# TheDisorderedOrganization/MonteCarlo

Hardware: AMD Instinct MI355X
Metric: chain-updates/sec (MC sweeps x M) at M=10^7 per MI355X (higher is better)
Workload: dtype f64

## Files before the change

montecarlo_amd/csrc/amc_api.hip:

```cpp
#include "amc_internal.h"

static thread_local std::string g_last_error;

int fail(int code, const char* fmt, ...)
{
    char buf[2048];
    va_list ap;
    va_start(ap, fmt);
    vsnprintf(buf, sizeof(buf), fmt, ap);
    va_end(ap);
    g_last_error = buf;
    return code;
}

int grid_for(const amc_handle* h, int64_t n_items, int blocks_per_cu)
{
    int64_t blocks = (n_items + AMC_BLOCK - 1) / AMC_BLOCK;
    const int64_t cap = (int64_t)h->n_cu * (blocks_per_cu > 0 ? blocks_per_cu : h->blocks_per_cu);
    if (blocks > cap) blocks = cap;
    if (blocks < 1) blocks = 1;
    return (int)blocks;
}

static int push_params(amc_handle* h, const double* sigma, const double* weight)
// ... 231 lines not shown
        if (e != hipErrorNotReady) return e;
        if ((spins & 63) == 63) {
            timespec t1;
            clock_gettime(CLOCK_MONOTONIC, &t1);
            if ((t1.tv_sec - t0.tv_sec) * 1000000000ll + (t1.tv_nsec - t0.tv_nsec) > 5000000ll) break;
        }
    }
    return hipStreamSynchronize(stream);
}

static hipError_t wait_event(hipEvent_t ev)
{
    timespec t0;
    clock_gettime(CLOCK_MONOTONIC, &t0);
    for (int spins = 0;; ++spins) {
        const hipError_t e = hipEventQuery(ev);
        if (e != hipErrorNotReady) return e;
        if ((spins & 63) == 63) {
            timespec t1;
            clock_gettime(CLOCK_MONOTONIC, &t1);
            if ((t1.tv_sec - t0.tv_sec) * 1000000000ll + (t1.tv_nsec - t0.tv_nsec) > 5000000ll) break;
        }
    }
    return hipEventSynchronize(ev);
}


extern "C" {

const char* amc_last_error(void) { return g_last_error.c_str(); }

int amc_version(void) { return AMC_VERSION_MAJOR * 1000 + AMC_VERSION_MINOR; }

int amc_device_count(int* count)
{
    if (!count) return fail(AMC_ERR_BAD_ARG, "amc_device_count: count is NULL");
    int n = 0;
    hipError_t e = hipGetDeviceCount(&n);
    if (e != hipSuccess) { *count = 0; return fail(AMC_ERR_NO_DEVICE, "hipGetDeviceCount: %s", hipGetErrorString(e)); }
    *count = n;
    return AMC_OK;
}

struct ClassExprs { const char *sample, *logq, *dlogq, *perform, *invert; };
struct ProposalExprs { const char *sample, *logq, *dlogq, *perform, *invert; int n_params; const char* const* dlogq_more;
                       int n_classes; const ClassExprs* more_classes; const int* class_of_move; };

static int validate_proposal_exprs(const ProposalExprs* proposal)
{
    int rc_p = validate_potential_expr(proposal->sample, "sample_action expression", "z");
    if (rc_p == AMC_OK) rc_p = validate_potential_expr(proposal->logq, "log_proposal_density expression", "delta");
    if (rc_p == AMC_OK && proposal->dlogq) {
        rc_p = validate_potential_expr(proposal->dlogq, "d log_proposal_density / d sigma expression", proposal->n_params > 1 ? "" : "sigma");
        if (rc_p != AMC_OK && proposal->n_params == 1 &&
            validate_potential_expr(proposal->dlogq, "d log_proposal_density / d sigma expression", "theta0") == AMC_OK)
            rc_p = AMC_OK;
    }
    for (int pidx = 1; rc_p == AMC_OK && proposal->dlogq && pidx < proposal->n_params; ++pidx)
        rc_p = validate_potential_expr(proposal->dlogq_more[pidx - 1], "d log_proposal_density / d theta expression", "");
    if (rc_p == AMC_OK && (proposal->perform != nullptr) != (proposal->invert != nullptr))
        rc_p = fail(AMC_ERR_BAD_ARG, "amc_create_action_model: perform_expr and invert_expr come together (No invert_action! is defined)");
    if (rc_p == AMC_OK && proposal->perform) rc_p = validate_potential_expr(proposal->perform, "perform_action expression", "delta");
    if (rc_p == AMC_OK && proposal->invert) rc_p = validate_potential_expr(proposal->invert, "invert_action expression", "delta");
    for (int c = 1; rc_p == AMC_OK && c < proposal->n_classes; ++c) {
        const ClassExprs& ce = proposal->more_classes[c - 1];
        rc_p = validate_potential_expr(ce.sample, "sample_action expression", "z");
// ... 85 lines not shown
    }
    if (std::fabs(wsum - 1.0) > 1.4901161193847656e-08)
        return fail(AMC_ERR_BAD_ARG, "amc_create: weights must sum to 1 (got %.17g)", wsum);
    if (cfg->n_moves > 1 && !cfg->per_chain_counters) {
    }

    int n_dev = 0;
    hipError_t e = hipGetDeviceCount(&n_dev);
    if (e != hipSuccess || n_dev < 1)
        return fail(AMC_ERR_NO_DEVICE, "amc_create: no HIP device (%s); this engine has no CPU path",
                    e != hipSuccess ? hipGetErrorString(e) : "count = 0");
    if (cfg->device < 0 || cfg->device >= n_dev)
        return fail(AMC_ERR_BAD_ARG, "amc_create: device %d out of range [0, %d)", cfg->device, n_dev);
    AMC_HIP(hipSetDevice(cfg->device));
    hipDeviceProp_t prop;
    AMC_HIP(hipGetDeviceProperties(&prop, cfg->device));

    amc_handle* h = new (std::nothrow) amc_handle();
    if (!h) return fail(AMC_ERR_OOM, "amc_create: host allocation failed");
    h->device = cfg->device;
    h->n_cu = prop.multiProcessorCount > 0 ? prop.multiProcessorCount : 256;
    {
        std::string arch(prop.gcnArchName);
        const size_t colon = arch.find(':');
        if (colon != std::string::npos) arch.erase(colon);
        if (!arch.empty()) h->arch = arch;
        if (h->arch != AMC_BUILD_ARCH) {
            delete h;
            return fail(AMC_ERR_NO_DEVICE, "amc_create: device %d is %s, this libamc.so was built for %s (make ARCH=%s)", cfg->device,
                        arch.c_str(), AMC_BUILD_ARCH, arch.c_str());
        }
    }
    h->blocks_per_cu = 8;
    h->blocks_per_cu_single = (cfg->n_moves == 1 && !cfg->per_chain_counters) ? 6 : (cfg->n_moves > 1 ? 7 : 8);
    if (const char* env = std::getenv("AMC_BLOCKS_PER_CU")) {
        const int v = std::atoi(env);
        if (v >= 1 && v <= 64) h->blocks_per_cu = h->blocks_per_cu_single = h->blocks_per_cu_pg = v;
    }
    if (const char* env = std::getenv("AMC_BLOCKS_PER_CU_SINGLE")) {
        const int v = std::atoi(env);
        if (v >= 1 && v <= 64) h->blocks_per_cu_single = v;
    }
    if (const char* env = std::getenv("AMC_BLOCKS_PER_CU_REDUCE")) {
        const int v = std::atoi(env);
        if (v >= 1 && v <= 64) h->blocks_per_cu_red = v;
    }
    if (const char* env = std::getenv("AMC_EXACT_ACCEPT")) h->exact_accept = std::atoi(env) != 0;
    if (const char* env = std::getenv("AMC_WIDE_RED_ROWS")) h->wide_red_rows = std::atoi(env) != 0;
    if (const char* env = std::getenv("AMC_SHARD_ROUTE_ON_ONE_RANK")) h->shard_route_one_rank = std::atoi(env) != 0;
    if (const char* env = std::getenv("AMC_NO_DEFERRED_UPDATE")) h->no_deferred_update = std::atoi(env) != 0;
    if (const char* env = std::getenv("AMC_CLASS_PER_MOVE")) h->class_per_move_forced = std::atoi(env) != 0;
    if (const char* env = std::getenv("AMC_NO_COLUMN_SKIP")) h->no_column_skip = std::atoi(env) != 0;
    if (const char* env = std::getenv("AMC_NP_SMALL_LAUNCHES")) h->np_small_launches = std::atoi(env) != 0;
    h->M = cfg->n_chains;
    h->M_pad = ((cfg->n_chains + AMC_PAD_DOUBLES + 255) / 256) * 256;
    h->offset = cfg->chain_offset;
    h->M_global = cfg->n_chains_global;
    h->potential = cfg->potential;
    h->f32 = state_dtype == AMC_DTYPE_F32;
    h->use_rtc = h->f32 || cfg->potential == AMC_POTENTIAL_CUSTOM;
    h->pot_expr = encode_model_expr(h->f32, potential_expr, reward_expr, scale_expr, proposal);
    if (potential_expr && scale_expr) h->scaled_policy = true;
    if (potential_expr && proposal) {
        if (proposal->n_classes > 1) {
            h->n_classes = proposal->n_classes;
            for (int k = 0; k < cfg->n_moves; ++k) h->class_of_move[k] = proposal->class_of_move[k];
        }
        h->script_policy = true;
        h->script_dlogq = proposal->dlogq != nullptr;
        h->n_params = proposal->n_params;
    }
    h->K = cfg->n_moves;
    h->sweepstep = cfg->sweepstep;
    h->counters = cfg->per_chain_counters != 0 || cfg->n_moves > 1;
    h->beta = cfg->beta;
    h->seed = cfg->seed;

    int rc = AMC_OK;
    auto bail = [&](int code) { amc_destroy(h); return code; };
#define AMC_TRY(call)                                                                   \
    do {                                                                                \
        hipError_t e2_ = (call);                                                        \
        if (e2_ != hipSuccess) {                                                        \
            rc = fail(e2_ == hipErrorOutOfMemory ? AMC_ERR_OOM : AMC_ERR_HIP,           \
                      "%s failed: %s", #call, hipGetErrorString(e2_));                  \
            return bail(rc);                                                            \
        }                                                                               \
    } while (0)

    if (cfg->stream) {
        h->stream = (hipStream_t)cfg->stream;
    } else {
        AMC_TRY(hipStreamCreateWithFlags(&h->stream, hipStreamNonBlocking));
// ... 1218 lines not shown
```

montecarlo_amd/csrc/amc_math.h:

```cpp
#pragma once

#ifndef __HIPCC_RTC__
#include <hip/hip_runtime.h>
#include <stdint.h>
#else
typedef unsigned char uint8_t;
typedef unsigned short uint16_t;
typedef int int32_t;
typedef unsigned int uint32_t;
typedef long int64_t;
typedef unsigned long uint64_t;
#endif

#include "amc_tables.h"

namespace amc {

enum : uint32_t { STREAM_INIT = 0, STREAM_METROPOLIS = 1, STREAM_ESTIMATOR = 2 };
enum : uint32_t { DRAW_NORMAL = 0, DRAW_ACCEPT = 1 };

struct u32x4 { uint32_t x, y, z, w; };

__device__ __forceinline__ void stage_math_tables(double* lds, int tid, int nthreads)
{
    for (int i = tid; i < TAB_DOUBLES; i += nthreads) {
        const double v = AMC_MATH_TABLES[i];
        lds[i] = (i >= TAB_LOG_LOGC && i < TAB_SINPI) ? -2.0 * v : v;
    }
    __syncthreads();
}

__device__ __forceinline__ u32x4 philox4x32_10(u32x4 c, uint32_t k0, uint32_t k1)
{
#pragma unroll
    for (int r = 0; r < 10; ++r) {
        const uint64_t m0 = (uint64_t)0xD2511F53u * c.x;
        const uint64_t m1 = (uint64_t)0xCD9E8D57u * c.z;
        u32x4 n;
        n.x = __builtin_amdgcn_bitop3_b32((uint32_t)(m1 >> 32), c.y, k0, 0x96);
        n.y = (uint32_t)m1;
        n.z = __builtin_amdgcn_bitop3_b32((uint32_t)(m0 >> 32), c.w, k1, 0x96);
        n.w = (uint32_t)m0;
        c = n;
        k0 += 0x9E3779B9u;
        k1 += 0xBB67AE85u;
#ifndef AMC_PHILOX_HOISTED_KEYS
        asm volatile("" : "+s"(k0), "+s"(k1));
#endif
    }
    return c;
}

__device__ __forceinline__ u32x4 draw_counter(uint64_t pair, uint64_t t, uint32_t draw, uint32_t stream)
{
    u32x4 c;
    c.x = (uint32_t)t;
    c.y = ((uint32_t)(t >> 32) & 0xFFFFu) | ((draw & 0xFFFu) << 16) | ((stream & 0xFu) << 28);
    c.z = (uint32_t)pair;
    c.w = (uint32_t)(pair >> 32);
    return c;
}

__device__ __forceinline__ double bits_to_binade(uint32_t lo, uint32_t hi, uint32_t expo_hi)
{
    const uint32_t w_hi = __builtin_amdgcn_alignbit(expo_hi, hi, 12);
    const uint32_t w_lo = __builtin_amdgcn_alignbit(hi, lo, 12);
    return __longlong_as_double((long long)(((uint64_t)w_hi << 32) | w_lo));
}

__device__ __forceinline__ double uniform_co(uint32_t lo, uint32_t hi) { return bits_to_binade(lo, hi, 0x3FFu) - 1.0; }
__device__ __forceinline__ double uniform_oc(uint32_t lo, uint32_t hi) { return 2.0 - bits_to_binade(lo, hi, 0x3FFu); }
__device__ __forceinline__ double angle28(uint32_t w)
{
    const uint32_t w_hi = __builtin_amdgcn_alignbit(0x400u, w, 12);
    const uint32_t w_lo = (w << 20) & 0xFF000000u;
    return 4.0 - __longlong_as_double((long long)(((uint64_t)w_hi << 32) | w_lo));
}

__device__ __forceinline__ uint32_t spare_accept12(const u32x4& n, int half) { return half ? ((n.z >> 12) & 0xFFFu) : (n.x & 0xFFFu); }
__device__ __forceinline__ uint32_t spare_pick12(const u32x4& n, int half) { return half ? ((n.z >> 24) | ((n.w & 0xFu) << 8)) : (n.z & 0xFFFu); }
__device__ __forceinline__ double uniform_accept(uint32_t accept12, uint32_t lo, uint32_t hi)
{
    const uint32_t w_hi = 0x3FF00000u | (accept12 << 8) | (hi >> 24);
    const uint32_t w_lo = __builtin_amdgcn_alignbit(hi, lo, 24);
    return __longlong_as_double((long long)(((uint64_t)w_hi << 32) | w_lo)) - 1.0;
}
__device__ __forceinline__ double uniform_pick(uint32_t pick12, uint32_t lo)
{
    return (double)(((uint64_t)pick12 << 24) | (uint64_t)(lo & 0xFFFFFFu)) * 0x1.0p-36;
}

__device__ __forceinline__ double exp_core_f64(double x, const double* T)
{
    const double INV_L = 0x1.71547652b82fep+5;
    const double L_HI = 0x1.62e42fee00000p-6;
    const double L_LO = 0x1.a39ef35793c76p-38;
    const double SHIFT = 0x1.8p52;
    const double t = __builtin_fma(x, INV_L, SHIFT);
    const double kd = t - SHIFT;
    const int32_t ki = (int32_t)(uint32_t)(uint64_t)__double_as_longlong(t);
    double r = __builtin_fma(-kd, L_HI, x);
    r = __builtin_fma(-kd, L_LO, r);
    double p = 0x1.6c16c16c16c17p-10;
    p = __builtin_fma(p, r, 0x1.1111111111111p-7);
    p = __builtin_fma(p, r, 0x1.5555555555555p-5);
    p = __builtin_fma(p, r, 0x1.5555555555555p-3);
    p = __builtin_fma(p, r, 0x1.0000000000000p-1);
    p = __builtin_fma(p, r, 1.0);
    p = __builtin_fma(p, r, 1.0);
    const double y = T[TAB_EXP2 + (ki & 31)] * p;
    const int32_t m = ki >> 5;
    const uint64_t yb = (uint64_t)__double_as_longlong(y);
    const uint32_t yh = (uint32_t)(yb >> 32) + ((uint32_t)m << 20);
    return __longlong_as_double((long long)(((uint64_t)yh << 32) | (yb & 0xffffffffull)));
}

__device__ __forceinline__ double exp_f64(double x, const double* T)
{
    double y = exp_core_f64(x, T);
    y = (x < -708.0) ? 0.0 : y;
    y = (x > 709.0) ? __builtin_huge_val() : y;
    y = (x != x) ? x : y;
    return y;
}

__device__ __forceinline__ double log_f64(double x)
{
    const double LN2_HI = 0x1.62e42fee00000p-1;
    const double LN2_LO = 0x1.a39ef35793c76p-33;
    const double x0 = x;
    int64_t k = 0;
    uint64_t ux = (uint64_t)__double_as_longlong(x);
    if (ux < 0x0010000000000000ull) {
        x = x * 0x1.0p54;
        ux = (uint64_t)__double_as_longlong(x);
        k = -54;
    }
    uint32_t hx = (uint32_t)(ux >> 32);
    k += (int64_t)(hx >> 20) - 1023;
// ... 123 lines not shown
```

montecarlo_amd/csrc/amc_model.h:

```cpp
#pragma once

#include "amc_math.h"
#include "amc_xsum.h"

#define AMC_MAX_MOVES 64
#define AMC_MAX_LEARN 8
#ifndef AMC_BLOCK
#define AMC_BLOCK 256
#endif
#define AMC_PAD_DOUBLES (2 * AMC_BLOCK + 8)

namespace amc {

enum { POT_HARMONIC = 0, POT_DOUBLE_WELL = 1, POT_CUSTOM = 2 };

#ifndef AMC_PLAIN_KERNELS
#define AMC_PLAIN_KERNELS 1
#endif
#ifndef AMC_KERNEL_LINKAGE
#define AMC_KERNEL_LINKAGE
#endif

#ifdef AMC_STATE_F32
typedef float real_t;
// ... 322 lines not shown
#endif
}
#endif
#undef amc_exp
#undef amc_log

template <int POT>
__device__ __forceinline__ real_t potential(real_t x, const double* T)
{
    if (POT == POT_CUSTOM) return user_potential(x, T);
    if (POT == POT_DOUBLE_WELL) {
        const real_t q = x * x - (real_t)1.0;
        return q * q;
    }
    return x * x;
}

struct Proposal {
    real_t delta, xn, dlogp;
};

template <int POT>
__device__ __forceinline__ Proposal propose(real_t x, real_t beta, double sigma, double z, const double* T)
{
    Proposal p;
    p.delta = (real_t)__builtin_fma(sigma, z, 0.0);
    const real_t e1 = potential<POT>(x, T);
    p.xn = x + p.delta;
    const real_t e2 = potential<POT>(p.xn, T);
    p.dlogp = ((-e2) * beta) - ((-e1) * beta);
    return p;
}

__device__ __forceinline__ bool accept_exact(real_t delta, real_t dlogp, double den, double rden, double logc, double u,
                                             const double* T)
{
    const double logq = div_by_const((double)(-(delta * delta)), den, rden) - logc;
    const double arg = ((double)dlogp + logq) - logq;
    const bool c_pos = arg >= 0.0, c_rng = arg >= -708.0, c_exp = exp_core_f64(arg, T) > u;
    return c_pos | (c_rng & c_exp);
}

#define AMC_FILTER_EPS 0x1.0p-16f
struct FilterCmp {
    bool pos, lo, hi;
};

__device__ __forceinline__ FilterCmp accept_filter(real_t dlogp, uint32_t k)
{
    const float t = (float)dlogp;
    const float ex = __builtin_amdgcn_exp2f(__builtin_fmaxf(t, -17.0f) * 0x1.715476p+0f);
    const float kf = (float)k;
    constexpr float SCALE = 4096.0f;
    const float lo1 = __builtin_fmaf(ex, (1.0f - AMC_FILTER_EPS) * SCALE, -1.0f);
    const float hi = ex * ((1.0f + AMC_FILTER_EPS) * SCALE);
    FilterCmp c;
    c.pos = t > 2e-12f;
    c.lo = lo1 > kf;
    c.hi = hi < kf;
    return c;
}

__device__ __forceinline__ FilterCmp accept_filter_arg(double arg, uint32_t k)
{
    const float t = (float)arg;
    const float ex = __builtin_amdgcn_exp2f(__builtin_fmaxf(t, -17.0f) * 0x1.715476p+0f);
    const float kf = (float)k;
    constexpr float SCALE = 4096.0f;
    const float lo1 = __builtin_fmaf(ex, (1.0f - AMC_FILTER_EPS) * SCALE, -1.0f);
    const float hi = ex * ((1.0f + AMC_FILTER_EPS) * SCALE);
    FilterCmp c;
    c.pos = arg >= 0.0;
// ... 116 lines not shown
            if (!have_pu) {
                asm volatile("" : "+v"(accept_ctr.z));
                pu = philox4x32_10(accept_ctr, key0, key1);
            }
            a0 = accept_exact_arg(s0.arg, uniform_accept(a0_12, pu.x, pu.y), T);
            a1 = accept_exact_arg(s1.arg, uniform_accept(a1_12, pu.z, pu.w), T);
        }
        xv.x = a0 ? s0.xn : s0.xr;
        xv.y = a1 ? s1.xn : s1.xr;
        m0 = __builtin_amdgcn_ballot_w64(a0);
        m1_out = __builtin_amdgcn_ballot_w64(a1);
        acc_bits = (a0 ? 1u : 0u) | (a1 ? 0x100u : 0u);
        return;
    }
#endif
    const Proposal p0 = propose<POT>(xv.x, b0, sg0, z0, T), p1 = propose<POT>(xv.y, b1, sg1, z1, T);
    const real_t xr0 = p0.xn + (-p0.delta), xr1 = p1.xn + (-p1.delta);
    const FilterCmp c0 = accept_filter(p0.dlogp, a0_12), c1 = accept_filter(p1.dlogp, a1_12);
#define AMC_B(c) __builtin_amdgcn_ballot_w64(c)
    const unsigned long long acc0 = AMC_B(c0.pos) | AMC_B(c0.lo), rej0 = AMC_B(c0.hi);
    const unsigned long long acc1 = AMC_B(c1.pos) | AMC_B(c1.lo), rej1 = AMC_B(c1.hi);
    const unsigned long long undecided = AMC_B(true) & ~((acc0 | rej0) & (acc1 | rej1));
#undef AMC_B
    if ((undecided | force_mask) != 0ull) {
        if (!have_pu) {
            asm volatile("" : "+v"(accept_ctr.z));
            pu = philox4x32_10(accept_ctr, key0, key1);
        }
        MoveExact e0 = m1, e1 = m1;
        if (MULTI) {
            e0.dn = s_tab[AMC_MAX_MOVES + k0]; e0.lc = s_tab[2 * AMC_MAX_MOVES + k0]; e0.rd = s_tab[4 * AMC_MAX_MOVES + k0];
            e1.dn = s_tab[AMC_MAX_MOVES + k1]; e1.lc = s_tab[2 * AMC_MAX_MOVES + k1]; e1.rd = s_tab[4 * AMC_MAX_MOVES + k1];
        }
        const bool a0 = accept_exact(p0.delta, p0.dlogp, e0.dn, e0.rd, e0.lc, uniform_accept(a0_12, pu.x, pu.y), T);
        const bool a1 = accept_exact(p1.delta, p1.dlogp, e1.dn, e1.rd, e1.lc, uniform_accept(a1_12, pu.z, pu.w), T);
        m0 = __builtin_amdgcn_ballot_w64(a0);
        m1_out = __builtin_amdgcn_ballot_w64(a1);
        xv.x = a0 ? p0.xn : xr0;
        xv.y = a1 ? p1.xn : xr1;
        acc_bits = (a0 ? 1u : 0u) | (a1 ? 0x100u : 0u);
    } else {
        const bool a0 = c0.pos | c0.lo, a1 = c1.pos | c1.lo;
        m0 = acc0;
        m1_out = acc1;
        xv.x = a0 ? p0.xn : xr0;
        xv.y = a1 ? p1.xn : xr1;
        acc_bits = (a0 ? 1u : 0u) | (a1 ? 0x100u : 0u);
    }
}

typedef uint32_t u32v4_t __attribute__((ext_vector_type(4)));

typedef uint32_t u32v2_t __attribute__((ext_vector_type(2)));

__device__ __forceinline__ real2 load_pair_block(const real_t* block_base)
{
    const __amdgpu_buffer_rsrc_t r = __builtin_amdgcn_make_buffer_rsrc((void*)block_base, 0, 0x7fffffff, 0x00020000);
    real2 d;
#ifdef AMC_STATE_F32
    const u32v2_t v = __builtin_amdgcn_raw_buffer_load_b64(r, threadIdx.x * 8, 0, 0);
    d.x = __uint_as_float(v.x);
    d.y = __uint_as_float(v.y);
#else
    const u32v4_t v = __builtin_amdgcn_raw_buffer_load_b128(r, threadIdx.x * 16, 0, 0);
    d.x = __longlong_as_double((long long)(((uint64_t)v.y << 32) | v.x));
    d.y = __longlong_as_double((long long)(((uint64_t)v.w << 32) | v.z));
#endif
    return d;
// ... 16 lines not shown
```

montecarlo_amd/csrc/amc_sweep.h:

```cpp
#pragma once

#include "amc_wave_sums.h"

namespace amc {

struct SweepArgs {
    real_t* x;
    const real_t* beta_arr;
    uint8_t* log;
    const double* ptab;
    const uint8_t* pick_tab;
    unsigned long long* acc_total;
    int64_t n_chains;
    int64_t m_stride;
    uint64_t pair0;
    uint64_t t0;
    int32_t n_steps;
    int32_t n_moves;
    uint32_t key0, key1;
    double beta;
    xs_word* red_partials;
    int32_t red_stride;
    int32_t red_cols;
    int32_t log_pos;
    int32_t exact_accept;
    int32_t n_slots;
};

struct StepDraws {
    u32x4 normal;
};

__device__ __forceinline__ StepDraws step_draws(const SweepArgs& a, uint64_t pair, uint64_t t)
{
    StepDraws d;
    d.normal = philox4x32_10(draw_counter(pair, t, DRAW_NORMAL, STREAM_METROPOLIS), a.key0, a.key1);
    return d;
// ... 52 lines not shown
        const u32x4 accept_ctr = draw_counter(pair, t, DRAW_ACCEPT, STREAM_METROPOLIS);
        double sg0 = sigma1, sg1 = sigma1;
        int k0 = 0, k1 = 0;
        u32x4 pu = {0u, 0u, 0u, 0u};
        bool have_pu = false;
        if (MULTI) {
            const uint32_t q0 = spare_pick12(dr.normal, 0), q1 = spare_pick12(dr.normal, 1);
            k0 = s_pick[q0];
            k1 = s_pick[q1];
            const bool open = ((k0 | k1) & 0x80) != 0;
            if ((__builtin_amdgcn_ballot_w64(open) | force_mask) != 0ull) {
                pu = philox4x32_10(accept_ctr, a.key0, a.key1);
                have_pu = true;
                k0 = categorical_walk(s_tab, K, uniform_pick(q0, pu.x));
                k1 = categorical_walk(s_tab, K, uniform_pick(q1, pu.z));
            }
            sg0 = s_tab[k0];
            sg1 = s_tab[k1];
        }
        double z0, z1;
        box_muller(dr.normal, z0, z1, s_math, mk);
        unsigned long long m0, m1m;
        uint32_t acc_bits;
        mh_pair<POT, MULTI>(xv, b0, b1, sg0, sg1, k0, k1, s_tab, m1, z0, z1, dr.normal, pu, have_pu, accept_ctr, a.key0,
                            a.key1, s_math, force_mask, acc_bits, m0, m1m, th1);
        if (!MULTI) wave_acc += __popcll(m0 & __builtin_amdgcn_ballot_w64(v0)) + __popcll(m1m & __builtin_amdgcn_ballot_w64(v1));
        if (LOG) {
            log_word = acc_bits | ((uint32_t)k0 << 1) | ((uint32_t)k1 << 9);
            if (!SINGLE && v0) store_log_pair<LOG>(a, a.log_pos + s, p, log_word);
        }
    }
}

template <int POT, bool MULTI, int LOG, bool BETA, bool SINGLE, int REDUCE = RED_FORM_NONE>
__global__ __launch_bounds__(AMC_BLOCK) void sweep_kernel(const SweepArgs a)
{
    static_assert(!MULTI || LOG, "K > 1 always keeps per-chain counters");
    constexpr bool RED_E = REDUCE == RED_FORM_E;
    constexpr int RNC = RedCols<POT, RED_E>::NC;
    RLanes<RNC> red;
    __shared__ xs::PartR s_red[REDUCE ? AMC_BLOCK / 64 : 1][RNC];
    if (REDUCE) r_init(red, s_red[threadIdx.x >> 6]);
    __shared__ double s_tab[MULTI ? (5 + AMC_SIGMA_MEMO) * AMC_MAX_MOVES : 1];
    __shared__ __attribute__((aligned(16))) uint8_t s_pick[MULTI ? AMC_PICK_CELLS : 16];
    __shared__ double s_math[TAB_DOUBLES];
    const int K = a.n_moves;
    if (MULTI) {
        stage_pick_table(s_pick, a.pick_tab);
        for (int i = threadIdx.x; i < K; i += AMC_BLOCK) {
            s_tab[0 * AMC_MAX_MOVES + i] = a.ptab[PT_SIGMA * AMC_MAX_MOVES + i];
            s_tab[1 * AMC_MAX_MOVES + i] = a.ptab[PT_DEN * AMC_MAX_MOVES + i];
            s_tab[2 * AMC_MAX_MOVES + i] = a.ptab[PT_LOGC * AMC_MAX_MOVES + i];
            s_tab[3 * AMC_MAX_MOVES + i] = a.ptab[PT_CUM * AMC_MAX_MOVES + i];
            s_tab[4 * AMC_MAX_MOVES + i] = a.ptab[PT_RDEN * AMC_MAX_MOVES + i];
            if (AMC_SIGMA_MEMO) s_tab[(AMC_SIGMA_MEMO ? 5 : 0) * AMC_MAX_MOVES + i] = log_f64(a.ptab[PT_SIGMA * AMC_MAX_MOVES + i]);
        }
    }
    const double sigma1 = a.ptab[PT_SIGMA * AMC_MAX_MOVES];
    const double den1 = a.ptab[PT_DEN * AMC_MAX_MOVES];
    const double logc1 = a.ptab[PT_LOGC * AMC_MAX_MOVES];
    const double rden1 = a.ptab[PT_RDEN * AMC_MAX_MOVES];
    UserTheta th1 = {0.0, 0.0, 0.0, 0.0, 0.0, 0.0};
#ifdef AMC_USER_LOGQ
    if (!MULTI) th1 = user_theta_uniform(a.ptab, 0);
#endif

    const int64_t n_pairs = (a.n_chains + 1) >> 1;
    const int64_t stride = (int64_t)gridDim.x * AMC_BLOCK;
    const int64_t first = (int64_t)blockIdx.x * AMC_BLOCK;
    unsigned long long wave_acc = 0;
    unsigned long long slots_before = 0;
    if (REDUCE && !LOG && !MULTI && threadIdx.x == 0)
        for (int sl = (int)blockIdx.x; sl < a.n_slots; sl += (int)gridDim.x) slots_before += a.acc_total[sl];

    auto load_x = [&](int64_t b) -> real2 { return load_pair_block(a.x + 2 * b); };
    auto load_b = [&](int64_t b) -> real2 { return load_pair_block(a.beta_arr + 2 * b); };
    real2 x_nxt = {(real_t)0.0, (real_t)0.0}, b_nxt = {(real_t)a.beta, (real_t)a.beta};
    if (first < n_pairs) {
        x_nxt = load_x(first);
        if (BETA) b_nxt = load_b(first);
    }
    constexpr bool AHEAD = SINGLE;
    StepDraws dr_nxt = {};
    if (AHEAD && first < n_pairs) dr_nxt = step_draws(a, a.pair0 + (uint64_t)(first + threadIdx.x), a.t0);
#ifdef AMC_USER_LOGQ
    stage_user_theta(a.ptab, MULTI);
#endif
    stage_math_tables(s_math, threadIdx.x, AMC_BLOCK);
    __builtin_amdgcn_s_waitcnt(0x0F70);
    real2 x_done = {(real_t)0.0, (real_t)0.0};
    uint32_t lw_done = 0;
    int64_t base_done = -1;
    int64_t base = first;
    for (; base + stride < n_pairs; base += stride) {
        const int64_t p = base + threadIdx.x;
        real2 xv = x_nxt;
        const real_t b0 = b_nxt.x, b1 = b_nxt.y;
        x_nxt = load_x(base + stride);
        if (BETA) b_nxt = load_b(base + stride);
        if (base_done >= 0) {
            store_pair_block_writethrough(a.x + 2 * base_done, x_done);
            if (LOG && SINGLE) store_log_pair<LOG>(a, a.log_pos, base_done + threadIdx.x, lw_done);
        }
        const StepDraws dr = dr_nxt;
        uint32_t lw = 0;
        pair_steps<POT, MULTI, LOG, SINGLE, AHEAD>(a, xv, b0, b1, a.pair0 + (uint64_t)p, p, true, true, s_tab, s_pick, s_math,
                                                   sigma1, den1, rden1, logc1, wave_acc, lw, &dr, math_k_literal(), th1);
        if (AHEAD) dr_nxt = step_draws(a, a.pair0 + (uint64_t)(p + stride), a.t0);
        if (REDUCE) {
            red_add_pair<POT, RED_E>(red, xv, true, true, s_math, s_red[threadIdx.x >> 6], a.red_cols);
        }
        x_done = xv;
        lw_done = lw;
        base_done = base;
    }
    if (base < n_pairs) {
        const int64_t p = base + threadIdx.x;
        const bool v0 = p < n_pairs;
        const bool v1 = v0 && (2 * p + 1 < a.n_chains);
        real2 xv = x_nxt;
        if (base_done >= 0) {
            store_pair_block_writethrough(a.x + 2 * base_done, x_done);
            if (LOG && SINGLE) store_log_pair<LOG>(a, a.log_pos, base_done + threadIdx.x, lw_done);
        }
        uint32_t lw = 0;
        pair_steps<POT, MULTI, LOG, SINGLE, AHEAD>(a, xv, b_nxt.x, b_nxt.y, a.pair0 + (uint64_t)(v0 ? p : 0), p, v0, v1,
                                                   s_tab, s_pick, s_math, sigma1, den1, rden1, logc1, wave_acc, lw, &dr_nxt, math_k_literal(), th1);
        if (v0) {
            store_pair_block_writethrough(a.x + 2 * base, xv);
            if (LOG && SINGLE) store_log_pair<LOG>(a, a.log_pos, p, lw);
        }
        if (REDUCE) red_add_pair<POT, RED_E>(red, xv, v0, v1, s_math, s_red[threadIdx.x >> 6], a.red_cols);
    }
    if (REDUCE)
        red_finish<POT, RED_E>(red, s_red, a.red_partials + (int64_t)blockIdx.x * a.red_stride, a.red_stride == RED_COMPACT_WORDS, a.red_cols);
    if (!MULTI) {
        __shared__ unsigned long long s_acc[AMC_BLOCK / 64];
        if ((threadIdx.x & 63) == 0) s_acc[threadIdx.x >> 6] = wave_acc;
        __syncthreads();
        if (threadIdx.x == 0) {
            unsigned long long t = 0;
            for (int w = 0; w < AMC_BLOCK / 64; ++w) t += s_acc[w];
            if (REDUCE && !LOG) {
                if (t != 0) __hip_atomic_fetch_add(a.acc_total + blockIdx.x, t, __ATOMIC_RELAXED, __HIP_MEMORY_SCOPE_AGENT);
                a.red_partials[(int64_t)blockIdx.x * a.red_stride + (a.red_stride == RED_COMPACT_WORDS ? (int)RED_COMPACT_SLOT : (int)RED_ROW_SLOT)] =
                    (xs_word)__double_as_longlong((double)(slots_before + t));
            } else if (t != 0) {
                __hip_atomic_fetch_add(a.acc_total + blockIdx.x, t, __ATOMIC_RELAXED, __HIP_MEMORY_SCOPE_AGENT);
            }
        }
    }
}

__device__ __forceinline__ unsigned long long add_block_accepts(unsigned long long* acc_total, unsigned long long wave_acc)
{
    __shared__ unsigned long long s_acc2[AMC_BLOCK / 64];
    if ((threadIdx.x & 63) == 0) s_acc2[threadIdx.x >> 6] = wave_acc;
    __syncthreads();
    unsigned long long t = 0;
    if (threadIdx.x == 0) {
        for (int w = 0; w < AMC_BLOCK / 64; ++w) t += s_acc2[w];
        if (t != 0) __hip_atomic_fetch_add(acc_total + blockIdx.x, t, __ATOMIC_RELAXED, __HIP_MEMORY_SCOPE_AGENT);
    }
    __syncthreads();
    return t;
}

#define AMC_FOLD_TILE (16 * AMC_BLOCK)
__device__ __forceinline__ uint4 load_counter_quad(const uint32_t* p) { return *reinterpret_cast<const uint4*>(p); }
__device__ __forceinline__ uint4 load_counter_quad(const uint16_t* p)
{
    const uint2 v = *reinterpret_cast<const uint2*>(p);
    return uint4{v.x & 0xFFFFu, v.x >> 16, v.y & 0xFFFFu, v.y >> 16};
}
__device__ __forceinline__ void store_counter_quad(uint32_t* p, uint4 v) { *reinterpret_cast<uint4*>(p) = v; }
__device__ __forceinline__ void store_counter_quad(uint16_t* p, uint4 v)
{
    *reinterpret_cast<uint2*>(p) = uint2{v.x | (v.y << 16), v.z | (v.w << 16)};
}

template <bool HIGH, typename CT>
__device__ __forceinline__ uint4 bump_counter_quad(CT* lo, uint16_t* hi, uint32_t w)
{
    uint4 v = load_counter_quad(lo);
// ... 172 lines not shown
```

montecarlo_amd/csrc/amc_tables.h:

```cpp
#pragma once
#ifndef __HIPCC_RTC__
#include <hip/hip_runtime.h>
#endif
namespace amc {
enum { TAB_EXP2 = 0, TAB_LOG_INVC = 32, TAB_LOG_LOGC = 161, TAB_SINPI = 290, TAB_COSPI = 418,
       TAB_DOUBLES = 546, TAB_LOG_IDX_MIN = 53 };
__device__ const double AMC_MATH_TABLES[546] = {
    0x1.0000000000000p+0, 0x1.059b0d3158574p+0, 0x1.0b5586cf9890fp+0, 0x1.11301d0125b51p+0,
    0x1.172b83c7d517bp+0, 0x1.1d4873168b9aap+0, 0x1.2387a6e756238p+0, 0x1.29e9df51fdee1p+0,
    0x1.306fe0a31b715p+0, 0x1.371a7373aa9cbp+0, 0x1.3dea64c123422p+0, 0x1.44e086061892dp+0,
    0x1.4bfdad5362a27p+0, 0x1.5342b569d4f82p+0, 0x1.5ab07dd485429p+0, 0x1.6247eb03a5585p+0,
    0x1.6a09e667f3bcdp+0, 0x1.71f75e8ec5f74p+0, 0x1.7a11473eb0187p+0, 0x1.82589994cce13p+0,
    0x1.8ace5422aa0dbp+0, 0x1.93737b0cdc5e5p+0, 0x1.9c49182a3f090p+0, 0x1.a5503b23e255dp+0,
    0x1.ae89f995ad3adp+0, 0x1.b7f76f2fb5e47p+0, 0x1.c199bdd85529cp+0, 0x1.cb720dcef9069p+0,
    0x1.d5818dcfba487p+0, 0x1.dfc97337b9b5fp+0, 0x1.ea4afa2a490dap+0, 0x1.f50765b6e4540p+0,
    0x1.6900000000000p+0, 0x1.6700000000000p+0, 0x1.6500000000000p+0, 0x1.6300000000000p+0,
    0x1.6180000000000p+0, 0x1.5f80000000000p+0, 0x1.5d80000000000p+0, 0x1.5b80000000000p+0,
    0x1.5a00000000000p+0, 0x1.5800000000000p+0, 0x1.5600000000000p+0, 0x1.5480000000000p+0,
    0x1.5280000000000p+0, 0x1.5100000000000p+0, 0x1.4f00000000000p+0, 0x1.4d80000000000p+0,
    0x1.4c00000000000p+0, 0x1.4a00000000000p+0, 0x1.4880000000000p+0, 0x1.4700000000000p+0,
    0x1.4500000000000p+0, 0x1.4380000000000p+0, 0x1.4200000000000p+0, 0x1.4080000000000p+0,
    0x1.3f00000000000p+0, 0x1.3d80000000000p+0, 0x1.3c00000000000p+0, 0x1.3a80000000000p+0,
    0x1.3900000000000p+0, 0x1.3780000000000p+0, 0x1.3600000000000p+0, 0x1.3480000000000p+0,
    0x1.3300000000000p+0, 0x1.3180000000000p+0, 0x1.3000000000000p+0, 0x1.2e80000000000p+0,
    0x1.2d80000000000p+0, 0x1.2c00000000000p+0, 0x1.2a80000000000p+0, 0x1.2900000000000p+0,
    0x1.2800000000000p+0, 0x1.2680000000000p+0, 0x1.2500000000000p+0, 0x1.2400000000000p+0,
    0x1.2280000000000p+0, 0x1.2180000000000p+0, 0x1.2000000000000p+0, 0x1.1f00000000000p+0,
    0x1.1d80000000000p+0, 0x1.1c80000000000p+0, 0x1.1b00000000000p+0, 0x1.1a00000000000p+0,
    0x1.1880000000000p+0, 0x1.1780000000000p+0, 0x1.1680000000000p+0, 0x1.1500000000000p+0,
    0x1.1400000000000p+0, 0x1.1300000000000p+0, 0x1.1180000000000p+0, 0x1.1080000000000p+0,
    0x1.0f80000000000p+0, 0x1.0e80000000000p+0, 0x1.0d00000000000p+0, 0x1.0c00000000000p+0,
    0x1.0b00000000000p+0, 0x1.0a00000000000p+0, 0x1.0900000000000p+0, 0x1.0780000000000p+0,
    0x1.0680000000000p+0, 0x1.0580000000000p+0, 0x1.0480000000000p+0, 0x1.0380000000000p+0,
    0x1.0280000000000p+0, 0x1.0180000000000p+0, 0x1.0000000000000p+0, 0x1.0000000000000p+0,
    0x1.fa00000000000p-1, 0x1.f600000000000p-1, 0x1.f200000000000p-1, 0x1.ef00000000000p-1,
    0x1.eb00000000000p-1, 0x1.e700000000000p-1, 0x1.e400000000000p-1, 0x1.e000000000000p-1,
    0x1.dd00000000000p-1, 0x1.d900000000000p-1, 0x1.d600000000000p-1, 0x1.d200000000000p-1,
    0x1.cf00000000000p-1, 0x1.cc00000000000p-1, 0x1.c900000000000p-1, 0x1.c600000000000p-1,
    0x1.c200000000000p-1, 0x1.bf00000000000p-1, 0x1.bc00000000000p-1, 0x1.b900000000000p-1,
    0x1.b600000000000p-1, 0x1.b300000000000p-1, 0x1.b100000000000p-1, 0x1.ae00000000000p-1,
// ... 107 lines not shown
```

Baseline: 335.9 billion.

## Overlap math-table staging with chain loads, pin exp constants, raise residency

The kernel prologue now issues the math-table global loads as 16-byte pairs at kernel start and writes them into LDS only after the first chain/beta loads are in flight, so the table staging overlaps the initial memory latency. The first-step random draws move after the barrier. Exp-core constants in the exact-accept path are forced into scalar registers via an inline-asm barrier, and single-move sweep kernels get a waves-per-EU hint of 7, with the default blocks-per-CU for the non-RTC single case raised from 6 to 7. Optional timestamp diagnostics compiled out by default are added. Higher residency may increase register pressure or spills.

Measured after the change: 335.7 billion (median of 4 runs). Within noise of the previous version (-0.1%).

```diff
diff --git a/montecarlo_amd/csrc/amc_api.hip b/montecarlo_amd/csrc/amc_api.hip
--- a/montecarlo_amd/csrc/amc_api.hip
+++ b/montecarlo_amd/csrc/amc_api.hip
@@ -287,6 +287,19 @@
 
 int amc_version(void) { return AMC_VERSION_MAJOR * 1000 + AMC_VERSION_MINOR; }
 
+#ifdef AMC_DIAG_STAMPS
+extern "C" __attribute__((visibility("default"))) int amc_diag_stamps_read(unsigned long long* out, int clear)
+{
+    const size_t bytes = sizeof(unsigned long long) * AMC_DIAG_WAVES * AMC_DIAG_POINTS;
+    if (out && hipMemcpyFromSymbol(out, HIP_SYMBOL(amc::amc_diag_stamps), bytes, 0, hipMemcpyDeviceToHost) != hipSuccess) return -1;
+    if (clear) {
+        void* p = nullptr;
+        if (hipGetSymbolAddress(&p, HIP_SYMBOL(amc::amc_diag_stamps)) != hipSuccess || hipMemset(p, 0, bytes) != hipSuccess) return -1;
+    }
+    return AMC_DIAG_WAVES * AMC_DIAG_POINTS;
+}
+#endif
+
 int amc_device_count(int* count)
 {
     if (!count) return fail(AMC_ERR_BAD_ARG, "amc_device_count: count is NULL");
@@ -438,7 +451,7 @@
         }
     }
     h->blocks_per_cu = 8;
-    h->blocks_per_cu_single = (cfg->n_moves == 1 && !cfg->per_chain_counters) ? 6 : (cfg->n_moves > 1 ? 7 : 8);
+    h->blocks_per_cu_single = (cfg->n_moves == 1 && !cfg->per_chain_counters) ? 7 : (cfg->n_moves > 1 ? 7 : 8);
     if (const char* env = std::getenv("AMC_BLOCKS_PER_CU")) {
         const int v = std::atoi(env);
         if (v >= 1 && v <= 64) h->blocks_per_cu = h->blocks_per_cu_single = h->blocks_per_cu_pg = v;
@@ -465,6 +478,8 @@
     h->potential = cfg->potential;
     h->f32 = state_dtype == AMC_DTYPE_F32;
     h->use_rtc = h->f32 || cfg->potential == AMC_POTENTIAL_CUSTOM;
+    if (h->use_rtc && cfg->n_moves == 1 && !cfg->per_chain_counters && !std::getenv("AMC_BLOCKS_PER_CU_SINGLE") && !std::getenv("AMC_BLOCKS_PER_CU"))
+        h->blocks_per_cu_single = 6;
     h->pot_expr = encode_model_expr(h->f32, potential_expr, reward_expr, scale_expr, proposal);
     if (potential_expr && scale_expr) h->scaled_policy = true;
     if (potential_expr && proposal) {
diff --git a/montecarlo_amd/csrc/amc_math.h b/montecarlo_amd/csrc/amc_math.h
--- a/montecarlo_amd/csrc/amc_math.h
+++ b/montecarlo_amd/csrc/amc_math.h
@@ -28,6 +28,28 @@
         lds[i] = (i >= TAB_LOG_LOGC && i < TAB_SINPI) ? -2.0 * v : v;
     }
     __syncthreads();
+}
+
+struct MathTablePairs { double2 p0, p1; };
+__device__ __forceinline__ MathTablePairs math_tables_load(int tid)
+{
+    static_assert(TAB_DOUBLES % 2 == 0 && TAB_DOUBLES / 2 <= 2 * 256, "two 16-byte pairs per thread of a 256-thread block");
+    MathTablePairs t;
+    const int i1 = tid + 256 < TAB_DOUBLES / 2 ? tid + 256 : TAB_DOUBLES / 2 - 1;
+    t.p0 = reinterpret_cast<const double2*>(AMC_MATH_TABLES)[tid];
+    t.p1 = reinterpret_cast<const double2*>(AMC_MATH_TABLES)[i1];
+    return t;
+}
+__device__ __forceinline__ void math_tables_store(double* lds, int tid, MathTablePairs t)
+{
+    auto scaled = [](double2 v, int i) {
+        v.x = (2 * i >= TAB_LOG_LOGC && 2 * i < TAB_SINPI) ? -2.0 * v.x : v.x;
+        v.y = (2 * i + 1 >= TAB_LOG_LOGC && 2 * i + 1 < TAB_SINPI) ? -2.0 * v.y : v.y;
+        return v;
+    };
+    const int i1 = tid + 256 < TAB_DOUBLES / 2 ? tid + 256 : TAB_DOUBLES / 2 - 1;
+    reinterpret_cast<double2*>(lds)[tid] = scaled(t.p0, tid);
+    reinterpret_cast<double2*>(lds)[i1] = scaled(t.p1, i1);
 }
 
 __device__ __forceinline__ u32x4 philox4x32_10(u32x4 c, uint32_t k0, uint32_t k1)
@@ -90,21 +112,29 @@
     return (double)(((uint64_t)pick12 << 24) | (uint64_t)(lo & 0xFFFFFFu)) * 0x1.0p-36;
 }
 
+template <bool HERE>
+__device__ __forceinline__ double k_here(double v)
+{
+    if (HERE) asm volatile("" : "+s"(v));
+    return v;
+}
+
+template <bool HERE = false>
 __device__ __forceinline__ double exp_core_f64(double x, const double* T)
 {
-    const double INV_L = 0x1.71547652b82fep+5;
-    const double L_HI = 0x1.62e42fee00000p-6;
-    const double L_LO = 0x1.a39ef35793c76p-38;
+    const double INV_L = k_here<HERE>(0x1.71547652b82fep+5);
+    const double L_HI = k_here<HERE>(0x1.62e42fee00000p-6);
+    const double L_LO = k_here<HERE>(0x1.a39ef35793c76p-38);
     const double SHIFT = 0x1.8p52;
     const double t = __builtin_fma(x, INV_L, SHIFT);
     const double kd = t - SHIFT;
     const int32_t ki = (int32_t)(uint32_t)(uint64_t)__double_as_longlong(t);
     double r = __builtin_fma(-kd, L_HI, x);
     r = __builtin_fma(-kd, L_LO, r);
-    double p = 0x1.6c16c16c16c17p-10;
-    p = __builtin_fma(p, r, 0x1.1111111111111p-7);
-    p = __builtin_fma(p, r, 0x1.5555555555555p-5);
-    p = __builtin_fma(p, r, 0x1.5555555555555p-3);
+    double p = k_here<HERE>(0x1.6c16c16c16c17p-10);
+    p = __builtin_fma(p, r, k_here<HERE>(0x1.1111111111111p-7));
+    p = __builtin_fma(p, r, k_here<HERE>(0x1.5555555555555p-5));
+    p = __builtin_fma(p, r, k_here<HERE>(0x1.5555555555555p-3));
     p = __builtin_fma(p, r, 0x1.0000000000000p-1);
     p = __builtin_fma(p, r, 1.0);
     p = __builtin_fma(p, r, 1.0);
diff --git a/montecarlo_amd/csrc/amc_model.h b/montecarlo_amd/csrc/amc_model.h
--- a/montecarlo_amd/csrc/amc_model.h
+++ b/montecarlo_amd/csrc/amc_model.h
@@ -378,12 +378,13 @@
     return p;
 }
 
+template <bool HERE = false>
 __device__ __forceinline__ bool accept_exact(real_t delta, real_t dlogp, double den, double rden, double logc, double u,
                                              const double* T)
 {
     const double logq = div_by_const((double)(-(delta * delta)), den, rden) - logc;
     const double arg = ((double)dlogp + logq) - logq;
-    const bool c_pos = arg >= 0.0, c_rng = arg >= -708.0, c_exp = exp_core_f64(arg, T) > u;
+    const bool c_pos = arg >= 0.0, c_rng = arg >= k_here<HERE>(-708.0), c_exp = exp_core_f64<HERE>(arg, T) > u;
     return c_pos | (c_rng & c_exp);
 }
 
@@ -566,8 +567,8 @@
             e0.dn = s_tab[AMC_MAX_MOVES + k0]; e0.lc = s_tab[2 * AMC_MAX_MOVES + k0]; e0.rd = s_tab[4 * AMC_MAX_MOVES + k0];
             e1.dn = s_tab[AMC_MAX_MOVES + k1]; e1.lc = s_tab[2 * AMC_MAX_MOVES + k1]; e1.rd = s_tab[4 * AMC_MAX_MOVES + k1];
         }
-        const bool a0 = accept_exact(p0.delta, p0.dlogp, e0.dn, e0.rd, e0.lc, uniform_accept(a0_12, pu.x, pu.y), T);
-        const bool a1 = accept_exact(p1.delta, p1.dlogp, e1.dn, e1.rd, e1.lc, uniform_accept(a1_12, pu.z, pu.w), T);
+        const bool a0 = accept_exact<true>(p0.delta, p0.dlogp, e0.dn, e0.rd, e0.lc, uniform_accept(a0_12, pu.x, pu.y), T);
+        const bool a1 = accept_exact<true>(p1.delta, p1.dlogp, e1.dn, e1.rd, e1.lc, uniform_accept(a1_12, pu.z, pu.w), T);
         m0 = __builtin_amdgcn_ballot_w64(a0);
         m1_out = __builtin_amdgcn_ballot_w64(a1);
         xv.x = a0 ? p0.xn : xr0;
diff --git a/montecarlo_amd/csrc/amc_sweep.h b/montecarlo_amd/csrc/amc_sweep.h
--- a/montecarlo_amd/csrc/amc_sweep.h
+++ b/montecarlo_amd/csrc/amc_sweep.h
@@ -3,6 +3,21 @@
 #include "amc_wave_sums.h"
 
 namespace amc {
+
+#ifdef AMC_DIAG_STAMPS
+#define AMC_DIAG_WAVES 16384
+#define AMC_DIAG_POINTS 6
+static __device__ unsigned long long amc_diag_stamps[AMC_DIAG_WAVES][AMC_DIAG_POINTS];
+#define AMC_DIAG_STAMP(i)                                                                                                  \
+    do {                                                                                                                   \
+        unsigned long long amc_t_;                                                                                         \
+        asm volatile("s_memrealtime %0\n\ts_waitcnt lgkmcnt(0)" : "=s"(amc_t_)::"memory");                               \
+        const unsigned amc_w_ = blockIdx.x * (AMC_BLOCK / 64) + (threadIdx.x >> 6);                                        \
+        if ((threadIdx.x & 63) == 0 && amc_w_ < AMC_DIAG_WAVES) amc_diag_stamps[amc_w_][(i)] = amc_t_;                      \
+    } while (0)
+#else
+#define AMC_DIAG_STAMP(i) do {} while (0)
+#endif
 
 struct SweepArgs {
     real_t* x;
@@ -121,8 +136,13 @@
     }
 }
 
+#ifndef __HIPCC_RTC__
+#define AMC_SWEEP_RESIDENCY(MULTI) __attribute__((amdgpu_waves_per_eu((MULTI) ? 1 : 7)))
+#else
+#define AMC_SWEEP_RESIDENCY(MULTI)
+#endif
 template <int POT, bool MULTI, int LOG, bool BETA, bool SINGLE, int REDUCE = RED_FORM_NONE>
-__global__ __launch_bounds__(AMC_BLOCK) void sweep_kernel(const SweepArgs a)
+__global__ __launch_bounds__(AMC_BLOCK) AMC_SWEEP_RESIDENCY(MULTI) void sweep_kernel(const SweepArgs a)
 {
     static_assert(!MULTI || LOG, "K > 1 always keeps per-chain counters");
     constexpr bool RED_E = REDUCE == RED_FORM_E;
@@ -132,7 +152,9 @@
     if (REDUCE) r_init(red, s_red[threadIdx.x >> 6]);
     __shared__ double s_tab[MULTI ? (5 + AMC_SIGMA_MEMO) * AMC_MAX_MOVES : 1];
     __shared__ __attribute__((aligned(16))) uint8_t s_pick[MULTI ? AMC_PICK_CELLS : 16];
-    __shared__ double s_math[TAB_DOUBLES];
+    __shared__ __attribute__((aligned(16))) double s_math[TAB_DOUBLES];
+    AMC_DIAG_STAMP(0);
+    const MathTablePairs mt = math_tables_load(threadIdx.x);
     const int K = a.n_moves;
     if (MULTI) {
         stage_pick_table(s_pick, a.pick_tab);
@@ -164,19 +186,27 @@
 
     auto load_x = [&](int64_t b) -> real2 { return load_pair_block(a.x + 2 * b); };
     auto load_b = [&](int64_t b) -> real2 { return load_pair_block(a.beta_arr + 2 * b); };
+    auto stage = [&]() {
+        math_tables_store(s_math, threadIdx.x, mt);
+#ifdef AMC_USER_LOGQ
+        stage_user_theta(a.ptab, MULTI);
+#endif
+        __syncthreads();
+        AMC_DIAG_STAMP(1);
+    };
+    constexpr bool AHEAD = SINGLE;
+    StepDraws dr_nxt = {};
     real2 x_nxt = {(real_t)0.0, (real_t)0.0}, b_nxt = {(real_t)a.beta, (real_t)a.beta};
     if (first < n_pairs) {
         x_nxt = load_x(first);
         if (BETA) b_nxt = load_b(first);
-    }
-    constexpr bool AHEAD = SINGLE;
-    StepDraws dr_nxt = {};
-    if (AHEAD && first < n_pairs) dr_nxt = step_draws(a, a.pair0 + (uint64_t)(first + threadIdx.x), a.t0);
-#ifdef AMC_USER_LOGQ
-    stage_user_theta(a.ptab, MULTI);
-#endif
-    stage_math_tables(s_math, threadIdx.x, AMC_BLOCK);
-    __builtin_amdgcn_s_waitcnt(0x0F70);
+        stage();
+        if (AHEAD) dr_nxt = step_draws(a, a.pair0 + (uint64_t)(first + threadIdx.x), a.t0);
+        __builtin_amdgcn_s_waitcnt(0x0F70);
+    } else {
+        stage();
+    }
+    AMC_DIAG_STAMP(2);
     real2 x_done = {(real_t)0.0, (real_t)0.0};
     uint32_t lw_done = 0;
     int64_t base_done = -1;
@@ -196,6 +226,9 @@
         pair_steps<POT, MULTI, LOG, SINGLE, AHEAD>(a, xv, b0, b1, a.pair0 + (uint64_t)p, p, true, true, s_tab, s_pick, s_math,
                                                    sigma1, den1, rden1, logc1, wave_acc, lw, &dr, math_k_literal(), th1);
         if (AHEAD) dr_nxt = step_draws(a, a.pair0 + (uint64_t)(p + stride), a.t0);
+#ifdef AMC_DIAG_STAMPS
+        if (base == first) AMC_DIAG_STAMP(3);
+#endif
         if (REDUCE) {
             red_add_pair<POT, RED_E>(red, xv, true, true, s_math, s_red[threadIdx.x >> 6], a.red_cols);
         }
@@ -203,6 +236,7 @@
         lw_done = lw;
         base_done = base;
     }
+    AMC_DIAG_STAMP(4);
     if (base < n_pairs) {
         const int64_t p = base + threadIdx.x;
         const bool v0 = p < n_pairs;
@@ -239,6 +273,7 @@
             }
         }
     }
+    AMC_DIAG_STAMP(5);
 }
 
 __device__ __forceinline__ unsigned long long add_block_accepts(unsigned long long* acc_total, unsigned long long wave_acc)
diff --git a/montecarlo_amd/csrc/amc_tables.h b/montecarlo_amd/csrc/amc_tables.h
--- a/montecarlo_amd/csrc/amc_tables.h
+++ b/montecarlo_amd/csrc/amc_tables.h
@@ -5,7 +5,7 @@
 namespace amc {
 enum { TAB_EXP2 = 0, TAB_LOG_INVC = 32, TAB_LOG_LOGC = 161, TAB_SINPI = 290, TAB_COSPI = 418,
        TAB_DOUBLES = 546, TAB_LOG_IDX_MIN = 53 };
-__device__ const double AMC_MATH_TABLES[546] = {
+__device__ __attribute__((aligned(16))) const double AMC_MATH_TABLES[546] = {
     0x1.0000000000000p+0, 0x1.059b0d3158574p+0, 0x1.0b5586cf9890fp+0, 0x1.11301d0125b51p+0,
     0x1.172b83c7d517bp+0, 0x1.1d4873168b9aap+0, 0x1.2387a6e756238p+0, 0x1.29e9df51fdee1p+0,
     0x1.306fe0a31b715p+0, 0x1.371a7373aa9cbp+0, 0x1.3dea64c123422p+0, 0x1.44e086061892dp+0,
```
